# kvas7andy/unreal

Hardware: AMD Instinct MI355X
Metric: env-steps/sec (whole node), UNREAL maze 84x84 (higher is better)
Workload: dtype f32 (fp16x2-split MFMA operands, fp32 accumulate)

## Files before the change

include/unreal_hip.h:

```cpp
#ifndef UNREAL_HIP_H
#define UNREAL_HIP_H
#include <stdint.h>
#ifdef __cplusplus
extern "C" {
#endif

#define UNREAL_FRAME_BYTES 21168
#define UNREAL_PC_CELLS 400
#define UNREAL_GEMM_RELU 1
#define UNREAL_GEMM_ACCUM 2
#define UNREAL_GEMM_ATOMIC 4
#define UNREAL_GEMM_RELU_MASK 8
#define UNREAL_GEMM_RELU_BITS 16

#define UNREAL_MAZE_NAV_RECORD 8
#define UNREAL_MAZE_GEN_RECORD(N) (8 + 18 + (N) * (N) + 65)
#define UNREAL_MAZE_TOP_DOWN 0
#define UNREAL_MAZE_FIRST_PERSON 1
#define UNREAL_MAZE_FIRST_PERSON_GENERATED 2
int unreal_maze_reset(int B, int H1, const int* mask, int* pos, int* last_action, float* last_reward, const int* count,
                      uint8_t* frames, int view, int N, const int* cfg, int actor_base, int* goal, int* layout,
                      int* ep_steps, int* episode, int* heading, void* stream);
int unreal_maze_step(int B, int H1, const int* actions, const int* active, int* pos, int* last_action, float* last_reward,
                     int* count, uint8_t* frames, float* r_reward, int* r_action, int* r_terminal, int* r_last_action,
// ... 99 lines not shown
int unreal_gemm_f32_split_nt(int M, int N, int K, const float* A, int lda, const float* a_absmax, const uint16_t* W2,
                             int ldw, long plane_stride, const float* w_absmax, float* C, int ldc, float* c_absmax,
                             const float* bias,
                             const void* mask ,
                             int ldm, int flags, int splitk, void* stream);
int unreal_gemm_f32_split_nt_slabs(int M, int N, int K, const float* A, int lda, const float* a_absmax, const uint16_t* W3,
                                   int ldw, long plane_stride, const float* w_absmax, float* C, int ldc, float* c_absmax,
                                   const float* bias, int flags, int splitk, float* partials, long partial_floats,
                                   void* stream);
int unreal_gemm_f32_split_tn(int M, int N, int K, const float* A, int lda, const float* a_absmax, const float* B, int ldb,
                             const float* b_absmax, float* C, int ldc, float* colsum, int splitk, void* stream);
int unreal_shadow_refresh_multi(const void* abs_descs, int n_abs, int abs_blocks, const void* split_descs, int n_split,
                                int split_blocks, void* stream);
int unreal_split_f16x2(int rows, int cols, const float* src, int ld_src, int transpose, int row_perm, uint16_t* dst,
                       int ld_dst, long plane_stride, const float* w_absmax, void* stream);
int unreal_lstm_step_fwd(int rows, const float* x, int ldx, int Kx, const float* x_absmax, const float* h_prev, int ld_hprev,
                         const uint16_t* W2, int ldw, long plane_stride, const float* w_absmax, float* gates,
                         const float* bias, const float* c_prev, float* c_out, float* h_out, int ld_h, void* stream);
int unreal_lstm_bptt_step(int rows, const float* d_gates, const float* a_absmax, const uint16_t* Wh2, int ldw,
                          long plane_stride, const float* w_absmax, const float* dh_above, float* dc_io,
                          const float* gates_act, const float* c_prev, const float* c_new, float* dpre,
                          float* dpre_absmax0, float* dpre_absmax1, void* stream);
int unreal_lstm_gates_fwd(int rows, const float* pre, const float* bias, const float* c_prev, float* gates_act,
                          float* c_out, float* h_out, int ld_h, void* stream);
int unreal_lstm_gates_bwd(int rows, const float* dh_above, const float* dh_rec, float* dc_io, const float* gates_act,
                          const float* c_prev, const float* c_new, float* dpre, float* dpre_absmax0 ,
                          float* dpre_absmax1 , void* stream);

int unreal_linear_small_fwd(int rows, int K, int NOUT, const float* X, int ldx, const float* W, const float* b,
                            float* out, int ldo, void* stream);
int unreal_linear_small_bwd(int rows, int K, int NOUT, const float* X, int ldx, const float* dO, int ldo,
                            const float* W, float* dX, int lddx, int accumulate_dx, float* dW, int dw_stride_k,
                            int dw_stride_n, float* db, void* stream);
int unreal_softmax_sample(int rows, int A, float* logits_pi, int ld, const double* u, int* action, void* stream);
int unreal_policy_step(int rows, int A, const float* X, int ldx, const float* Wp, const float* bp, const float* Wv,
                       const float* bv, const double* u, float* pi_out, float* v_out, int* action, void* stream);
int unreal_base_loss_grad(int rows, int A, const float* pi, int ld_pi, const float* v, const int* action,
                          const float* adv, const float* R, const int* active, float entropy_beta, float grad_scale,
                          float* dlogits, float* dv, float* losses , void* stream);
int unreal_vr_loss_grad(int rows, const float* v, const float* R, const int* mask, float grad_scale, float* dv,
                        float* loss, void* stream);
int unreal_rp_loss_grad(int rows, const float* logits, const int* cls, float grad_scale, float* prob, float* dlogits,
                        float* loss, void* stream);
int unreal_colsum(int rows, int cols, const float* X, int ld, float* out, void* stream);
int unreal_relu_mask(int rows, int cols, float* d, int ldd, const float* src, int lds, void* stream);

int unreal_pc_deconv_fwd(int N, int A, const float* hp, const float* hp_absmax, const float* Wv, const float* bv,
                         const float* Wa, const float* ba, float* qmax, const int* action, const float* target,
                         const int* mask, float lambda, float grad_scale, float* d_dec, float* ddec_absmax, float* loss,
                         void* stream);
int unreal_pc_deconv_bwd(int N, int A, const float* hp, const float* hp_absmax, const float* d_dec, const float* ddec_absmax,
                         const float* Wv, const float* Wa, float* d_hp, float* dhp_absmax ,
                         float* dWv, float* dbv, float* dWa, float* dba, void* stream);
int unreal_pc_deconv_train(int N, int A, const float* hp, const float* hp_absmax, const float* Wv, const float* bv,
                           const float* Wa, const float* ba, const int* action, const float* target, const int* mask,
                           float lambda, float grad_scale, float* loss, float* d_hp,
                           float* dhp_absmax , float* dWv, float* dbv, float* dWa,
                           float* dba, float* d_dec, void* stream);

int unreal_grad_norm(const float* grad, long n, float* scratch , float* norm_out, void* stream);
int unreal_rmsprop_step(float* var, float* ms, float* mom, const float* grad, long n, float lr, float decay,
                        float momentum, float eps, float clip_norm, const float* norm, void* stream);

int unreal_copy_words(long n, const void* src, void* dst, void* stream);
int unreal_axpy_f32(long n, float alpha, const float* x, float* y, void* stream);
int unreal_last_launch(char* buf, int len, void* stream);
// ... 6 lines not shown
```

unreal_amd/csrc/heads.hip:

```cpp
#include "common.h"
#include "policy_row.h"

namespace {

__device__ __forceinline__ float sigmoidf_(float x) { return 1.f / (1.f + expf(-x)); }

__global__ void lstm_gates_fwd_kernel(int rows, const float* __restrict__ pre, const float* __restrict__ bias,
                                      const float* __restrict__ c_prev, float* __restrict__ gates_act,
                                      float* __restrict__ c_out, float* __restrict__ h_out, int ld_h) {
  int g = blockIdx.x * blockDim.x + threadIdx.x;
  if (g >= rows * LSTM_N) return;
  int r = g / LSTM_N, u = g - r * LSTM_N;
  const float* p = pre + (size_t)r * 4 * LSTM_N;
  float i = sigmoidf_(p[u] + bias[u]);
  float j = tanhf(p[LSTM_N + u] + bias[LSTM_N + u]);
  float f = sigmoidf_(p[2 * LSTM_N + u] + bias[2 * LSTM_N + u] + 1.0f);
  float o = sigmoidf_(p[3 * LSTM_N + u] + bias[3 * LSTM_N + u]);
  float c = c_prev[g] * f + i * j;
  float h = tanhf(c) * o;
  if (gates_act) {
    float* ga = gates_act + (size_t)r * 4 * LSTM_N;
    ga[u] = i; ga[LSTM_N + u] = j; ga[2 * LSTM_N + u] = f; ga[3 * LSTM_N + u] = o;
  }
  c_out[g] = c;
  h_out[(size_t)r * ld_h + u] = h;
}

__global__ void lstm_gates_bwd_kernel(int rows, const float* __restrict__ dh_above, const float* __restrict__ dh_rec,
                                      float* __restrict__ dc_io, const float* __restrict__ gates_act,
                                      const float* __restrict__ c_prev, const float* __restrict__ c_new,
                                      float* __restrict__ dpre, float* absmax0, float* absmax1) {
  float m = 0.f;
// ... 6 lines not shown
  float dc = dc_io[g] + dh * o * (1.f - tc * tc);
  float* d = dpre + (size_t)r * 4 * LSTM_N;
  const float d0 = dc * j * i * (1.f - i), d1 = dc * i * (1.f - j * j), d2 = dc * c_prev[g] * f * (1.f - f),
              d3 = dh * tc * o * (1.f - o);
  d[u] = d0;
  d[LSTM_N + u] = d1;
  d[2 * LSTM_N + u] = d2;
  d[3 * LSTM_N + u] = d3;
  dc_io[g] = dc * f;
  m = fmaxf(fmaxf(m, fmaxf(fabsf(d0), fabsf(d1))), fmaxf(fabsf(d2), fabsf(d3)));
  }
  __shared__ float wmx[4];
  m = wave_max(m);
  if ((threadIdx.x & 63) == 0) wmx[threadIdx.x >> 6] = m;
  __syncthreads();
  if (threadIdx.x < 64) {
    const float mm = fmaxf(fmaxf(wmx[0], wmx[1]), fmaxf(wmx[2], wmx[3]));
    absmax_commit(absmax0, mm);
    absmax_commit(absmax1, mm);
  }
}

template <int NOUT>
__global__ __launch_bounds__(256) void linear_small_fwd_kernel(int rows, int K, const float* __restrict__ X, int ldx,
                                                               const float* __restrict__ W, const float* __restrict__ b,
                                                               float* __restrict__ out, int ldo) {
  int row = blockIdx.x * 4 + (threadIdx.x >> 6);
  int lane = threadIdx.x & 63;
  if (row >= rows) return;
  float acc[NOUT];
#pragma unroll
  for (int n = 0; n < NOUT; ++n) acc[n] = 0.f;
  const float* x = X + (size_t)row * ldx;
  for (int k = lane; k < K; k += 64) {
    float xv = x[k];
#pragma unroll
    for (int n = 0; n < NOUT; ++n) acc[n] += xv * W[(size_t)k * NOUT + n];
  }
#pragma unroll
  for (int n = 0; n < NOUT; ++n) acc[n] = wave_sum(acc[n]);
  if (lane == 0)
#pragma unroll
    for (int n = 0; n < NOUT; ++n) out[(size_t)row * ldo + n] = acc[n] + b[n];
}

template <int NOUT>
__global__ __launch_bounds__(256) void linear_small_bwd_kernel(int rows, int K, int rows_per_block,
                                                               const float* __restrict__ X, int ldx,
                                                               const float* __restrict__ dO, int ldo,
                                                               const float* __restrict__ W, float* __restrict__ dX,
                                                               int lddx, int accumulate_dx, float* __restrict__ dW,
                                                               int dw_sk, int dw_sn, float* __restrict__ db) {
  const int k = blockIdx.x * 256 + threadIdx.x;
  const int r0 = blockIdx.y * rows_per_block;
  const int nr = min(rows_per_block, rows - r0);
  if (k >= K) return;
  float w[NOUT], acc[NOUT], sdb[NOUT];
#pragma unroll
  for (int n = 0; n < NOUT; ++n) { w[n] = W ? W[(size_t)k * NOUT + n] : 0.f; acc[n] = 0.f; sdb[n] = 0.f; }
  int r = 0;
  for (; r + 4 <= nr; r += 4) {
    float xv[4], old[4], d[4][NOUT];
#pragma unroll
    for (int u = 0; u < 4; ++u) xv[u] = X[(size_t)(r0 + r + u) * ldx + k];
    if (dX && accumulate_dx) {
#pragma unroll
      for (int u = 0; u < 4; ++u) old[u] = dX[(size_t)(r0 + r + u) * lddx + k];
    }
#pragma unroll
    for (int u = 0; u < 4; ++u)
// ... 2 lines not shown
#pragma unroll
    for (int u = 0; u < 4; ++u) {
      float dx = 0.f;
#pragma unroll
      for (int n = 0; n < NOUT; ++n) {
        acc[n] += xv[u] * d[u][n];
        dx += d[u][n] * w[n];
        sdb[n] += d[u][n];
      }
      if (dX) dX[(size_t)(r0 + r + u) * lddx + k] = accumulate_dx ? (old[u] + dx) : dx;
    }
  }
  for (; r < nr; ++r) {
    const size_t row = (size_t)(r0 + r);
    float xv = X[row * ldx + k];
    float dx = 0.f;
#pragma unroll
    for (int n = 0; n < NOUT; ++n) {
      const float d = dO[row * ldo + n];
      acc[n] += xv * d;
      dx += d * w[n];
      sdb[n] += d;
    }
    if (dX) {
      float* p = dX + row * lddx + k;
      *p = accumulate_dx ? (*p + dx) : dx;
    }
  }
#pragma unroll
  for (int n = 0; n < NOUT; ++n) atomicAdd(dW + (size_t)k * dw_sk + (size_t)n * dw_sn, acc[n]);
  if (db && k == 0) {
#pragma unroll
    for (int n = 0; n < NOUT; ++n) atomicAdd(db + n, sdb[n]);
  }
}

__global__ void softmax_sample_kernel(int rows, int A, float* __restrict__ logits_pi, int ld, const double* __restrict__ u,
                                      int* __restrict__ action) {
  int r = blockIdx.x * blockDim.x + threadIdx.x;
  if (r >= rows) return;
  float* p = logits_pi + (size_t)r * ld;
  float m = p[0];
  for (int a = 1; a < A; ++a) m = fmaxf(m, p[a]);
  float s = 0.f;
  for (int a = 0; a < A; ++a) { float e = expf(p[a] - m); p[a] = e; s += e; }
  for (int a = 0; a < A; ++a) p[a] = p[a] / s;
  if (action && u) {
    double tot = 0.0;
    for (int a = 0; a < A; ++a) tot += (double)p[a];
    double run = 0.0, uu = u[r];
    int act = 0;
    for (int a = 0; a < A; ++a) {
      run += (double)p[a];
      if (run / tot <= uu) act = a + 1;
    }
    action[r] = min(act, A - 1);
  } else if (action) {
    int best = 0;
    for (int a = 1; a < A; ++a)
      if (p[a] > p[best]) best = a;
    action[r] = best;
  }
}

template <int A>
__global__ __launch_bounds__(256) void policy_step_kernel(int rows, const float* __restrict__ X, int ldx,
// ... 114 lines not shown
  }
  part[ry][cx] = (s0 + s1) + (s2 + s3);
  __syncthreads();
  if (ry == 0 && c < cols) atomicAdd(out + c, (part[0][cx] + part[1][cx]) + (part[2][cx] + part[3][cx]));
}

__global__ void relu_mask_kernel(int rows, int cols, float* __restrict__ d, int ldd, const float* __restrict__ src, int lds) {
  int g = blockIdx.x * blockDim.x + threadIdx.x;
  if (g >= rows * cols) return;
  int r = g / cols, c = g - r * cols;
  float* p = d + (size_t)r * ldd + c;
  if (!(src[(size_t)r * lds + c] > 0.f)) *p = 0.f;
}

template <int NOUT>
int launch_small_fwd(int rows, int K, const float* X, int ldx, const float* W, const float* b, float* out, int ldo,
                     hipStream_t st) {
  hipLaunchKernelGGL((linear_small_fwd_kernel<NOUT>), dim3((rows + 3) / 4), dim3(256), 0, st, rows, K, X, ldx, W, b, out,
                     ldo);
  return unreal_launch_status();
}

template <int NOUT>
int launch_small_bwd(int rows, int K, const float* X, int ldx, const float* dO, int ldo, const float* W, float* dX,
                     int lddx, int acc, float* dW, int dw_sk, int dw_sn, float* db, hipStream_t st) {
  if (dw_sk == 0 && dw_sn == 0) { dw_sk = NOUT; dw_sn = 1; }
  const int rpb = 128;
  dim3 grid((K + 255) / 256, (rows + rpb - 1) / rpb);
  hipLaunchKernelGGL((linear_small_bwd_kernel<NOUT>), grid, dim3(256), 0, st, rows, K, rpb, X,
                     ldx, dO, ldo, W, dX, lddx, acc, dW, dw_sk, dw_sn, db);
  return unreal_launch_status();
}

}

#define GRID1(n) dim3(((n) + 255) / 256), dim3(256), 0, (hipStream_t)stream

extern "C" {

int unreal_lstm_gates_fwd(int rows, const float* pre, const float* bias, const float* c_prev, float* gates_act,
                          float* c_out, float* h_out, int ld_h, void* stream) {
  if (rows <= 0 || !pre || !bias || !c_prev || !c_out || !h_out || ld_h < LSTM_N) return UNREAL_EINVAL;
  hipLaunchKernelGGL(lstm_gates_fwd_kernel, GRID1(rows * LSTM_N), rows, pre, bias, c_prev, gates_act, c_out, h_out,
                     ld_h);
  return unreal_launch_status();
}

int unreal_lstm_gates_bwd(int rows, const float* dh_above, const float* dh_rec, float* dc_io, const float* gates_act,
                          const float* c_prev, const float* c_new, float* dpre, float* dpre_absmax0, float* dpre_absmax1,
                          void* stream) {
  if (rows <= 0 || !dh_above || !dc_io || !gates_act || !c_prev || !c_new || !dpre) return UNREAL_EINVAL;
  hipLaunchKernelGGL(lstm_gates_bwd_kernel, dim3(min(rows, 1024)), dim3(256), 0, (hipStream_t)stream, rows, dh_above, dh_rec,
                     dc_io, gates_act, c_prev, c_new, dpre, dpre_absmax0, dpre_absmax1);
  return unreal_launch_status();
}

int unreal_linear_small_fwd(int rows, int K, int NOUT, const float* X, int ldx, const float* W, const float* b,
                            float* out, int ldo, void* stream) {
  if (rows <= 0 || K <= 0 || !X || !W || !b || !out || ldx < K || ldo < NOUT) return UNREAL_EINVAL;
  hipStream_t st = (hipStream_t)stream;
  switch (NOUT) {
#define SMALL_FWD(n) case n: return launch_small_fwd<n>(rows, K, X, ldx, W, b, out, ldo, st);
    SMALL_FWD(1) SMALL_FWD(3) SMALL_FWD(4) SMALL_FWD(6)
    SMALL_FWD(2) SMALL_FWD(5) SMALL_FWD(7) SMALL_FWD(8) SMALL_FWD(9)
    SMALL_FWD(10) SMALL_FWD(11) SMALL_FWD(12) SMALL_FWD(13) SMALL_FWD(14) SMALL_FWD(15) SMALL_FWD(16) SMALL_FWD(17)
    SMALL_FWD(18) SMALL_FWD(19)
#undef SMALL_FWD
    default: return UNREAL_EINVAL;
  }
}

int unreal_linear_small_bwd(int rows, int K, int NOUT, const float* X, int ldx, const float* dO, int ldo,
                            const float* W, float* dX, int lddx, int accumulate_dx, float* dW, int dw_stride_k,
                            int dw_stride_n, float* db, void* stream) {
  if (rows <= 0 || K <= 0 || !X || !dO || !dW || ldx < K || ldo < NOUT) return UNREAL_EINVAL;
  if (dX && !W) return UNREAL_EINVAL;
  hipStream_t st = (hipStream_t)stream;
  switch (NOUT) {
#define SMALL_BWD(n) \
    case n: return launch_small_bwd<n>(rows, K, X, ldx, dO, ldo, W, dX, lddx, accumulate_dx, dW, dw_stride_k, dw_stride_n, db, st);
    SMALL_BWD(1) SMALL_BWD(3) SMALL_BWD(4) SMALL_BWD(5) SMALL_BWD(6) SMALL_BWD(7)
    SMALL_BWD(2) SMALL_BWD(8) SMALL_BWD(9) SMALL_BWD(10) SMALL_BWD(11) SMALL_BWD(12) SMALL_BWD(13)
    SMALL_BWD(14) SMALL_BWD(15) SMALL_BWD(16) SMALL_BWD(17) SMALL_BWD(18) SMALL_BWD(19)
#undef SMALL_BWD
    default: return UNREAL_EINVAL;
  }
}

int unreal_softmax_sample(int rows, int A, float* logits_pi, int ld, const double* u, int* action, void* stream) {
  if (rows <= 0 || A <= 0 || A > UNREAL_MAX_ACTIONS || !logits_pi || ld < A) return UNREAL_EINVAL;
  hipLaunchKernelGGL(softmax_sample_kernel, GRID1(rows), rows, A, logits_pi, ld, u, action);
  return unreal_launch_status();
}

int unreal_policy_step(int rows, int A, const float* X, int ldx, const float* Wp, const float* bp, const float* Wv,
                       const float* bv, const double* u, float* pi_out, float* v_out, int* action, void* stream) {
  if (rows <= 0 || !X || !Wp || !bp || !Wv || !bv || !pi_out || !v_out || !action || ldx < LSTM_N) return UNREAL_EINVAL;
  hipStream_t st = (hipStream_t)stream;
  dim3 grid((rows + 3) / 4), block(256);
  switch (A) {
#define POLICY_STEP(a) \
    case a: hipLaunchKernelGGL((policy_step_kernel<a>), grid, block, 0, st, rows, X, ldx, Wp, bp, Wv, bv, u, pi_out, v_out, action); break;
    POLICY_STEP(3) POLICY_STEP(4) POLICY_STEP(6)
    POLICY_STEP(2) POLICY_STEP(5) POLICY_STEP(7) POLICY_STEP(8) POLICY_STEP(9) POLICY_STEP(10)
    POLICY_STEP(11) POLICY_STEP(12) POLICY_STEP(13) POLICY_STEP(14) POLICY_STEP(15) POLICY_STEP(16) POLICY_STEP(17)
    POLICY_STEP(18)
#undef POLICY_STEP
    default: return UNREAL_EINVAL;
  }
  return unreal_launch_status();
}

int unreal_base_loss_grad(int rows, int A, const float* pi, int ld_pi, const float* v, const int* action,
                          const float* adv, const float* R, const int* active, float entropy_beta, float grad_scale,
                          float* dlogits, float* dv, float* losses, void* stream) {
  if (rows <= 0 || A <= 0 || A > UNREAL_MAX_ACTIONS || !pi || !v || !action || !adv || !R || !active || !dlogits || !dv ||
      !losses)
    return UNREAL_EINVAL;
  if (A <= 8)
    hipLaunchKernelGGL(base_loss_grad_kernel<8>, GRID1(rows), rows, A, pi, ld_pi, v, action, adv, R, active, entropy_beta,
                       grad_scale, dlogits, dv, losses);
// ... 36 lines not shown
```

unreal_amd/csrc/replay.hip:

```cpp
#include "common.h"

namespace {

__global__ void sample_seq_kernel(int B, int H, int H1, int L, const int* start_draw, const int* count,
                                  const int* r_terminal, int* seq_idx, int* seq_len) {
  int b = blockIdx.x * blockDim.x + threadIdx.x;
  if (b >= B) return;
  const int cnt = count[b];
  const int top = max(0, cnt - H);
  int a0 = top + start_draw[b];
  const size_t rb = (size_t)b * H1;
  if (r_terminal[rb + a0 % H1]) a0 += 1;
  int n = 0, last = 0;
  for (int i = 0; i < L; ++i) {
    int a = min(a0 + i, cnt - 1);
    int idx = (int)(rb + a % H1);
    seq_idx[(size_t)i * B + b] = idx;
    last = idx;
    ++n;
    if (r_terminal[idx]) break;
  }
  for (int i = n; i < L; ++i) seq_idx[(size_t)i * B + b] = last;
  seq_len[b] = n;
}
// ... 33 lines not shown
    int pc = __popcll(m);
    if (run + pc > rank) {
      int k = rank - run;
      int before = __popcll(m & ((1ull << lane) - 1ull));
      unsigned long long hit = __ballot(member && before == k);
      end = lo + c + (__ffsll((long long)hit) - 1);
      break;
    }
    run += pc;
  }
  if (lane < 3) rp_idx[b * 3 + lane] = (int)(rb + (end - 3 + lane) % H1);
  if (lane == 0) {
    float r = r_reward[rb + end % H1];
    rp_class[b] = (r > -1e-10f && r < 1e-10f) ? 0 : (r > 0.f ? 1 : 2);
  }
}

__global__ void base_returns_kernel(int B, int T, const float* rewards, const float* values, const int* n_steps,
                                    const float* boot_v, const int* terminal_end, double gamma, float* R_out,
                                    float* adv_out) {
  int b = blockIdx.x * blockDim.x + threadIdx.x;
  if (b >= B) return;
  const int n = n_steps[b];
  double R = terminal_end[b] ? 0.0 : (double)boot_v[b];
  for (int t = T - 1; t >= 0; --t) {
    size_t i = (size_t)t * B + b;
    if (t >= n) { R_out[i] = 0.f; adv_out[i] = 0.f; continue; }
    R = (double)rewards[i] + gamma * R;
    R_out[i] = (float)R;
    adv_out[i] = (float)(R - (double)values[i]);
  }
}

__global__ void vr_returns_kernel(int B, int L, const int* seq_idx, const int* seq_len, const float* r_reward,
                                  const int* r_terminal, const float* boot_v, double gamma, float* R_out) {
  int b = blockIdx.x * blockDim.x + threadIdx.x;
  if (b >= B) return;
  const int n = seq_len[b];
  double R = (n >= 2 && r_terminal[seq_idx[(size_t)(n - 2) * B + b]]) ? 0.0 : (double)boot_v[b];
  for (int t = L - 2; t >= 0; --t) {
    size_t i = (size_t)t * B + b;
    if (t >= n - 1) { R_out[i] = 0.f; continue; }
    R = (double)r_reward[seq_idx[i]] + gamma * R;
    R_out[i] = (float)R;
  }
}

__global__ void pc_returns_kernel(int B, int L, const int* seq_idx, const int* seq_len, const float* r_pc,
                                  const int* r_terminal, const float* boot_qmax, double gamma_pc, float* R_out) {
  int g = blockIdx.x * blockDim.x + threadIdx.x;
  if (g >= B * PC_CELLS) return;
  const int b = g / PC_CELLS, c = g - b * PC_CELLS;
  const int n = seq_len[b];
  double R = (n >= 2 && r_terminal[seq_idx[(size_t)(n - 2) * B + b]]) ? 0.0 : (double)boot_qmax[g];
  for (int t = L - 2; t >= 0; --t) {
    size_t row = (size_t)t * B + b;
    if (t >= n - 1) { R_out[row * PC_CELLS + c] = 0.f; continue; }
    R = (double)r_pc[(size_t)seq_idx[row] * PC_CELLS + c] + gamma_pc * R;
    R_out[row * PC_CELLS + c] = (float)R;
  }
}

__global__ void lar_fill_kernel(int rows, int A, const int* last_action, const float* last_reward, const int* idx,
                                float* xcat, int ld, int col0, int clip) {
  int g = blockIdx.x * blockDim.x + threadIdx.x;
  const int w = ld - col0;
  if (g >= rows * w) return;
  int r = g / w, k = g - r * w;
  int src = idx ? idx[r] : r;
  float v = 0.f;
  if (k < A) v = (last_action[src] == k) ? 1.f : 0.f;
  else if (k == A) v = clip ? fminf(fmaxf(last_reward[src], -1.f), 1.f) : last_reward[src];
  xcat[(size_t)r * ld + col0 + k] = v;
}

__global__ void objective_put_kernel(int B, int H1, int obj, const int* count, const int* active, const float* staged,
                                     float* r_objective) {
  int g = blockIdx.x * blockDim.x + threadIdx.x;
  if (g >= B * obj) return;
  int b = g / obj, j = g - b * obj;
  if (active && !active[b]) return;
  r_objective[((size_t)b * H1 + count[b] % H1) * obj + j] = staged[g];
}

__global__ void objective_fill_kernel(int rows, int obj, int H1, const float* r_objective, const int* idx, int slot_offset,
                                      float* xcat, int ld, int col0) {
  int g = blockIdx.x * blockDim.x + threadIdx.x;
  if (g >= rows * obj) return;
  int r = g / obj, j = g - r * obj;
  int f = idx[r], b = f / H1, s = f - b * H1;
  s = (s + slot_offset % H1 + H1) % H1;
  xcat[(size_t)r * ld + col0 + j] = r_objective[((size_t)b * H1 + s) * obj + j];
// ... 178 lines not shown
```

unreal_amd/ops.py:

```python
import torch

from ._lib import lib, ptr, stream

FRAME_BYTES = 21168
PC_CELLS = 400
F2_DIM = 2592
C1_DIM = 6400
GEMM_RELU, GEMM_ACCUM, GEMM_ATOMIC, GEMM_RELU_MASK, GEMM_RELU_BITS = 1, 2, 4, 8, 16
RELU_WORDS = 162

FRAME_SHAPE = (84, 84)
FRAME_HW_MIN, FRAME_HW_MAX = 20, 480


def frame_dims(H, W):
    H, W = int(H), int(W)
    if not (FRAME_HW_MIN <= H <= FRAME_HW_MAX and FRAME_HW_MIN <= W <= FRAME_HW_MAX):
        raise ValueError("frame size %dx%d: supported are %d <= H, W <= %d" % (H, W, FRAME_HW_MIN, FRAME_HW_MAX))
    h1, w1 = (H - 8) // 4 + 1, (W - 8) // 4 + 1
    h2, w2 = (h1 - 4) // 2 + 1, (w1 - 4) // 2 + 1
    return h1, w1, h2, w2, 32 * h2 * w2


def frame_stride(H, W):
# ... 712 lines not shown


def lstm_bptt_step(rows, d_gates, Wh, dh_above, dc_io, gates_act, c_prev, c_new, dpre, a_max=None, c_max0=None,
                   c_max1=None):
    if Wh.N != 256 or Wh.K != 1024 or getattr(Wh, "row_perm", 0):
        raise ValueError("lstm_bptt_step needs the natural [256,1024] shadow of the recurrent kernel rows")
    _chk(d_gates, "f32", rows * 1024, "d_gates"); _chk(dh_above, "f32", rows * 256); _chk(dc_io, "f32", rows * 256)
    _chk(gates_act, "f32", rows * 1024); _chk(c_prev, "f32", rows * 256); _chk(c_new, "f32", rows * 256)
    _chk(dpre, "f32", rows * 1024)
    _chk(a_max, "f32", 1, "a_max", optional=True); _chk(c_max0, "f32", 1, "c_max0", optional=True)
    _chk(c_max1, "f32", 1, "c_max1", optional=True)
    a_max = _absmax_of(d_gates, rows, 1024, 1024, a_max)
    _call("unreal_lstm_bptt_step", rows, ptr(d_gates), ptr(a_max), ptr(Wh.planes), Wh.ldw, Wh.plane, ptr(Wh.wmax),
          ptr(dh_above), ptr(dc_io), ptr(gates_act), ptr(c_prev), ptr(c_new), ptr(dpre), ptr(c_max0), ptr(c_max1))


def linear_small_fwd(rows, K, NOUT, X, ldx, W, b, out, ldo):
    _chk(X, "f32", (rows - 1) * ldx + K); _chk(W, "f32", K * NOUT); _chk(b, "f32", NOUT)
    _chk(out, "f32", (rows - 1) * ldo + NOUT)
    _call("unreal_linear_small_fwd", rows, K, NOUT, ptr(X), ldx, ptr(W), ptr(b), ptr(out), ldo)


def linear_small_bwd(rows, K, NOUT, X, ldx, dO, ldo, W, dX, lddx, accumulate_dx, dW, db, dw_stride_k=0, dw_stride_n=0):
    _chk(X, "f32", (rows - 1) * ldx + K); _chk(dO, "f32", (rows - 1) * ldo + NOUT)
    _chk(W, "f32", K * NOUT, optional=dX is None)
    _chk(dX, "f32", (rows - 1) * lddx + K, optional=True)
    sk, sn = (dw_stride_k, dw_stride_n) if (dw_stride_k or dw_stride_n) else (NOUT, 1)
    _chk(dW, "f32", (K - 1) * sk + (NOUT - 1) * sn + 1)
    _chk(db, "f32", NOUT, optional=True)
    _call("unreal_linear_small_bwd", rows, K, NOUT, ptr(X), ldx, ptr(dO), ldo, ptr(W), ptr(dX), lddx,
          int(accumulate_dx), ptr(dW), int(dw_stride_k), int(dw_stride_n), ptr(db))


def policy_step(rows, A, X, ldx, Wp, bp, Wv, bv, u, pi_out, v_out, action):
    _chk(X, "f32", (rows - 1) * ldx + 256, "X"); _chk(Wp, "f32", 256 * A); _chk(bp, "f32", A); _chk(Wv, "f32", 256)
    _chk(bv, "f32", 1); _chk(u, "f64", rows, "u", optional=True); _chk(pi_out, "f32", rows * A); _chk(v_out, "f32", rows)
    _chk(action, "i32", rows)
    _call("unreal_policy_step", rows, A, ptr(X), ldx, ptr(Wp), ptr(bp), ptr(Wv), ptr(bv), ptr(u), ptr(pi_out), ptr(v_out),
          ptr(action))


def softmax_sample(rows, A, logits_pi, ld, u=None, action=None):
    _chk(logits_pi, "f32", (rows - 1) * ld + A); _chk(u, "f64", rows, optional=True)
    _chk(action, "i32", rows, optional=True)
    _call("unreal_softmax_sample", rows, A, ptr(logits_pi), ld, ptr(u), ptr(action))


def base_loss_grad(rows, A, pi, ld_pi, v, action, adv, R, active, beta, grad_scale, dlogits, dv, losses):
    _chk(pi, "f32", (rows - 1) * ld_pi + A); _chk(v, "f32", rows); _chk(action, "i32", rows)
    _chk(adv, "f32", rows); _chk(R, "f32", rows); _chk(active, "i32", rows)
    _chk(dlogits, "f32", rows * A); _chk(dv, "f32", rows); _chk(losses, "f32", 3)
    _call("unreal_base_loss_grad", rows, A, ptr(pi), ld_pi, ptr(v), ptr(action), ptr(adv), ptr(R), ptr(active),
          float(beta), float(grad_scale), ptr(dlogits), ptr(dv), ptr(losses))


def vr_loss_grad(rows, v, R, mask, grad_scale, dv, loss):
    _chk(v, "f32", rows); _chk(R, "f32", rows); _chk(mask, "i32", rows); _chk(dv, "f32", rows); _chk(loss, "f32", 1)
    _call("unreal_vr_loss_grad", rows, ptr(v), ptr(R), ptr(mask), float(grad_scale), ptr(dv), ptr(loss))


def rp_loss_grad(rows, logits, cls, grad_scale, prob, dlogits, loss):
    _chk(logits, "f32", rows * 3); _chk(cls, "i32", rows); _chk(prob, "f32", rows * 3, optional=True)
    _chk(dlogits, "f32", rows * 3); _chk(loss, "f32", 1)
    _call("unreal_rp_loss_grad", rows, ptr(logits), ptr(cls), float(grad_scale), ptr(prob), ptr(dlogits), ptr(loss))


# ... 75 lines not shown
```

unreal_amd/train/trainer.py:

```python
import time

import torch

from .. import ops
from ..environment.environment import Environment
from ..environment.maze_environment import batched_maze_environment
from ..model.model import UnrealModel, PathWS, GradWS
from .experience import Experience

PERFORMANCE_LOG_INTERVAL = 2000


def log_uniform(lo, hi, rate):
    import math
    return math.exp(math.log(lo) * (1 - rate) + math.log(hi) * rate)


class PhiloxDraws(object):

    def __init__(self, seed, rank=0, batch=None, world_size=1):
        self.seed = int(seed)
        self.counter = 1
        self.batch = None if batch is None else int(batch)
        self.stride = None if batch is None else int(batch) * int(world_size)
# ... 384 lines not shown
                    nxt = dict(next_idx=ws.frame_idx[(t + 1) * B:(t + 2) * B])
                    if self.use_lstm:
                        nxt.update(next_lar=ws.xcat[(t + 1) * B * ws.xld:], lar_ld=ws.xld, lar_col0=256, A=A)
                if fuse_policy:
                    self.environment.policy_rollout_step(net, feat, ld, self.u_act[s], self.pi[t * B * A:(t + 1) * B * A],
                                                         self.v[s], self.actions[s], self.rewards[s], self.terminals[s],
                                                         self.active, self.active_log[s], self.n_steps, self.terminal_end,
                                                         **nxt)
                    continue
                self.environment.rollout_step(self.actions[s], self.rewards[s], self.terminals[s], self.active,
                                              self.active_log[s], self.n_steps, self.terminal_end, **nxt)
                continue
            self.environment.process(self.actions[s], self.active, self.rewards[s], self.terminals[s],
                                     reset_on_terminal=True, track_score=True)
            ops.rollout_advance(B, self.terminals[s], self.active, self.active_log[s], self.n_steps,
                                self.terminal_end)
        if self.use_lstm:
            ops.copy_(self.lstm_c, ws.c[(T - 1) * B * 256:T * B * 256])
            ops.copy_(self.lstm_h, ws.h[(T - 1) * B * 256:T * B * 256])
        bw = self.boot_ws
        if self.use_lstm:
            ops.copy_(bw.c0, self.lstm_c)
            ops.copy_(bw.h0, self.lstm_h)
        self.ring.cur_idx(out=bw.frame_idx[:B])
        feat, ld = net.trunk_forward(self.ring, bw, 1, B, lar_from_ring=False, save_c1=False,
                                     clip_lar=self.rp_mode == 1,
                                     objective_slot_offset=-1)
        net.value_forward(B, feat, ld, self.boot_v)
        if self.use_lstm:
            ops.reset_state(B, self.terminal_end, self.lstm_c, self.lstm_h)
        ops.base_returns(B, T, self.rewards, self.v, self.n_steps, self.boot_v, self.terminal_end, self.gamma,
                         self.R, self.adv)

    def _train_base(self):
        B, T, A, ws, net, g, p = self.Bg, self.n_step_TD, self.action_size, self.base_ws, self.local_network, \
            self.local_network.g, self.local_network.p
        rows = T * B
        ops.base_loss_grad(rows, A, self.pi, A, self.v, self.actions, self.adv, self.R, self.active_log,
                           self.entropy_beta, self.grad_scale, self.dlogits, self.dv, self.losses[0:3])
        feat, ld = net.features(ws)
        d_feat = self.gws.d_feat
        ops.linear_small_bwd(rows, 256, A, feat, ld, self.dlogits, A, p["W_base_fc_p"], d_feat, 256, False,
                             g["W_base_fc_p"], g["b_base_fc_p"])
        ops.linear_small_bwd(rows, 256, 1, feat, ld, self.dv, 1, p["W_base_fc_v"], d_feat, 256, True,
                             g["W_base_fc_v"], g["b_base_fc_v"])
        net.trunk_backward(self.ring, ws, self.gws, T, B, d_feat, h0_nonzero=True)

    def _sample_sequence(self):
        B, Ta, net = self.Bg, self.local_t_max, self.local_network
        L = Ta + 1
        self.draws.randint(self.experience_history_size - L - 1, self.seq_start)
        ops.replay_sample_seq(self.ring, L, self.seq_start, self.seq_idx, self.seq_len)
        bw = self.boot_ws
        ops.seq_last_idx(B, self.seq_idx, self.seq_len, bw.frame_idx[:B])
        if self.use_lstm:
            bw.c0.zero_()
            bw.h0.zero_()
        feat, ld = net.trunk_forward(self.ring, bw, 1, B, lar_from_ring=True, save_c1=False)
        return feat, ld

    def _aux_forward(self):
        B, Ta, net, ws = self.Bg, self.local_t_max, self.local_network, self.aux_ws
        rows = Ta * B
        ops.copy_(ws.frame_idx[:rows], self.seq_idx[:rows])
        if self.use_lstm:
            ws.c0.zero_()
            ws.h0.zero_()
        ops.seq_mask(B, Ta, self.seq_len, self.seq_mask)
        return net.trunk_forward(self.ring, ws, Ta, B, lar_from_ring=True, save_c1=True)

    fuse_pc_deconv = True
    keep_d_dec = False

    def _pc_deconv_loss_backward(self, gws, rows, mask, d_hp, s_hp):
        A, net = self.action_size, self.local_network
        p, g = net.p, net.g
        s_dhp = net.new_slot()
        if self.fuse_pc_deconv:
# ... 64 lines not shown
            ops.replay_sample_seq(self.ring, L, self.seq_start2[s], self.seq_idx2[s], self.seq_len2[s])
            ops.seq_last_idx(B, self.seq_idx2[s], self.seq_len2[s], self.last2[s * B:(s + 1) * B])
            ops.seq_mask(B, Ta, self.seq_len2[s], self.seq_mask2[s])
        bw = self.boot2_ws
        ops.gather_i32(self.last2, self.map_boot, bw.frame_idx[:2 * B])
        feat, ld = net.trunk_forward(self.ring, bw, 1, 2 * B, lar_from_ring=True, save_c1=False)
        s_bhp = net.new_slot()
        net.pc_head_forward(B, feat, 2 * ld, self.boot_hp, ws=self.boot2_ws, hp_max=s_bhp)
        ops.pc_deconv_fwd(B, A, self.boot_hp, p["W_pc_deconv_v"], p["b_pc_deconv_v"], p["W_pc_deconv_a"],
                          p["b_pc_deconv_a"], qmax=self.boot_qmax, hp_max=s_bhp)
        ops.pc_returns(self.ring, L, self.seq_idx2[0], self.seq_len2[0], self.boot_qmax, self.gamma_pc, gws.pc_R)
        net.value_forward(B, feat[ld:], 2 * ld, self.aux_boot_v)
        ops.vr_returns(self.ring, L, self.seq_idx2[1], self.seq_len2[1], self.aux_boot_v, self.gamma, self.aux_R)
        ws = self.aux2_ws
        ops.gather_i32(self.seq_idx_cat, self.map_seq, ws.frame_idx[:2 * rows])
        feat, ld = net.trunk_forward(self.ring, ws, Ta, 2 * B, lar_from_ring=True, save_c1=True)
        d_feat = gws.d_feat
        s_hp = net.new_slot()
        net.pc_head_forward(rows, feat, 2 * ld, gws.hp, ws=self.aux2_ws, hp_max=s_hp)
        ops.gather_i32(self.ring.r_action, self.seq_idx2[0][:rows], self.seq_act)
        d_hp = gws.d_hp
        s_dhp = self._pc_deconv_loss_backward(gws, rows, self.seq_mask2[0], d_hp, s_hp)
        from ..model.model import _splitk
        ops.gemm_split_tn(256, 2592, rows, feat, 2 * ld, d_hp, 2592, g["W_pc_fc1"], 2592,
                          splitk=_splitk(256, 2592, rows), colsum=g["b_pc_fc1"],
                          a_max=net._one if self.use_lstm else self.aux2_ws.s_x, b_max=s_dhp)
        ops.gemm_split_nt(rows, 256, 2592, d_hp, 2592, sh["pc_fc1_dgrad"], d_feat, 2 * 256, a_max=s_dhp)
        net.value_forward(rows, feat[ld:], 2 * ld, self.aux_v)
        ops.vr_loss_grad(rows, self.aux_v, self.aux_R, self.seq_mask2[1], self.grad_scale, self.aux_dv, self.losses[4:5])
        ops.linear_small_bwd(rows, 256, 1, feat[ld:], 2 * ld, self.aux_dv, 1, p["W_base_fc_v"], d_feat[256:], 2 * 256, False,
                             g["W_base_fc_v"], g["b_base_fc_v"])
        net.trunk_backward(self.ring, ws, gws, Ta, 2 * B, d_feat)

    def _train_rp(self):
        B, net, ws = self.Bg, self.local_network, self.rp_ws
        p, g, gws = net.p, net.g, self.gws
        self.draws.randint(2, self.rp_coin)
        self.draws.uniform(self.rp_u)
        ops.replay_sample_rp(self.ring, self.rp_coin, self.rp_u, ws.frame_idx[:3 * B], self.rp_class, self.rp_mode)
        s_c1 = net.new_slot()
        F = net.F
        net.encoder_forward(self.ring, ws.frame_idx[:3 * B], ws.f2, ws.c1, c1_max=s_c1, ws=ws)
        ops.linear_small_fwd(B, 3 * F, 3, ws.f2, 3 * F, p["W_rp_fc1"], p["b_rp_fc1"], self.rp_logits, 3)
        ops.rp_loss_grad(B, self.rp_logits, self.rp_class, self.grad_scale, None, self.rp_dlogits,
                         self.losses[5:6])
        ops.linear_small_bwd(B, 3 * F, 3, ws.f2, 3 * F, self.rp_dlogits, 3, p["W_rp_fc1"], gws.d_f2, 3 * F, False,
                             g["W_rp_fc1"], g["b_rp_fc1"])
        ops.relu_mask(3 * B, F, gws.d_f2, F, ws.f2, F)
        net.encoder_backward(self.ring, ws.frame_idx[:3 * B], ws.c1, gws.d_f2,
                             c1_max=s_c1)

    def compute_gradients(self):
        net = self.local_network
        net.refresh_shadows()
        net.begin_pass()
        self._rollout()
        net.grads.flat.zero_()
        self.losses.zero_()
        self._train_base()
        if self.batch_aux:
            self._train_aux_batched()
        else:
            if self.use_pixel_change:
                self._train_pc()
            if self.use_value_replay:
                self._train_vr()
        if self.use_reward_prediction:
            self._train_rp()

    def process(self, sess=None, global_t=0, summary_writer=None, summary_op_dict=None, score_input=None,
                sr_input=None, eval_input=None, entropy_input=None, term_global_t=None, losses_input=None,
                sync_stats=True):
        if self.environment is None:
            self.prepare()
        if not self._full:
            self._fill_experience(sess)
            return 0, None
        net = self.local_network
# ... 63 lines not shown
```

Before: 3.711 million.

## Fuse small-head backward passes, unroll linear_small_fwd, and prefetch returns loads

Adds a one-pass small-linear backward kernel. It computes the policy and value head gradients together, and for the reward-prediction head it folds in the ReLU mask and the dx absmax. Both trainer paths are switched to it by default. This removes separate launches and repeated reads of the features. The forward small-linear loop is also unrolled with grouped loads. The returns kernels now prefetch chunks of reward loads before running the serial recurrence. The risks are changed fp summation order in dx and a new dependency on encoder_backward accepting a d2_max argument.

```diff
diff --git a/include/unreal_hip.h b/include/unreal_hip.h
--- a/include/unreal_hip.h
+++ b/include/unreal_hip.h
@@ -155,6 +155,12 @@
 int unreal_linear_small_bwd(int rows, int K, int NOUT, const float* X, int ldx, const float* dO, int ldo,
                             const float* W, float* dX, int lddx, int accumulate_dx, float* dW, int dw_stride_k,
                             int dw_stride_n, float* db, void* stream);
+int unreal_linear_small_bwd2(int rows, int K, int n1, int n2, const float* X, int ldx, const float* dO1, int ldo1,
+                             const float* W1, float* dW1, float* db1 , const float* dO2, int ldo2,
+                             const float* W2, float* dW2, float* db2 , float* dX, int lddx, void* stream);
+int unreal_linear_small_bwd_relu(int rows, int K, int NOUT, const float* X, int ldx, const float* dO, int ldo,
+                                 const float* W, float* dX, int lddx, float* dW, float* db ,
+                                 float* dx_absmax, void* stream);
 int unreal_softmax_sample(int rows, int A, float* logits_pi, int ld, const double* u, int* action, void* stream);
 int unreal_policy_step(int rows, int A, const float* X, int ldx, const float* Wp, const float* bp, const float* Wv,
                        const float* bv, const double* u, float* pi_out, float* v_out, int* action, void* stream);
diff --git a/unreal_amd/csrc/heads.hip b/unreal_amd/csrc/heads.hip
--- a/unreal_amd/csrc/heads.hip
+++ b/unreal_amd/csrc/heads.hip
@@ -1,3 +1,5 @@
+#include <type_traits>
+
 #include "common.h"
 #include "policy_row.h"
 
@@ -70,10 +72,25 @@
 #pragma unroll
   for (int n = 0; n < NOUT; ++n) acc[n] = 0.f;
   const float* x = X + (size_t)row * ldx;
-  for (int k = lane; k < K; k += 64) {
+  constexpr int U = NOUT <= 4 ? 8 : (NOUT <= 8 ? 4 : 1);
+  int k = lane;
+  for (; k + (U - 1) * 64 < K; k += U * 64) {
+    float xv[U], wv[U][NOUT];
+#pragma unroll
+    for (int u = 0; u < U; ++u) xv[u] = x[k + 64 * u];
+#pragma unroll
+    for (int u = 0; u < U; ++u)
+#pragma unroll
+      for (int n = 0; n < NOUT; ++n) wv[u][n] = W[(size_t)(k + 64 * u) * NOUT + n];
+#pragma unroll
+    for (int u = 0; u < U; ++u)
+#pragma unroll
+      for (int n = 0; n < NOUT; ++n) acc[n] = __builtin_fmaf(xv[u], wv[u][n], acc[n]);
+  }
+  for (; k < K; k += 64) {
     float xv = x[k];
 #pragma unroll
-    for (int n = 0; n < NOUT; ++n) acc[n] += xv * W[(size_t)k * NOUT + n];
+    for (int n = 0; n < NOUT; ++n) acc[n] = __builtin_fmaf(xv, W[(size_t)k * NOUT + n], acc[n]);
   }
 #pragma unroll
   for (int n = 0; n < NOUT; ++n) acc[n] = wave_sum(acc[n]);
@@ -142,6 +159,111 @@
   if (db && k == 0) {
 #pragma unroll
     for (int n = 0; n < NOUT; ++n) atomicAdd(db + n, sdb[n]);
+  }
+}
+
+template <int N, bool TAIL_ROW>
+__device__ __forceinline__ float small_bwd_dx(const float* d, const float* w) {
+#pragma clang fp contract(off)
+  constexpr int NF = TAIL_ROW ? N : (N > 12 ? N - 12 : 0);
+  float dx = 0.f;
+#pragma unroll
+  for (int n = 0; n < N; ++n) {
+    if (n < NF) {
+      dx = __builtin_fmaf(d[n], w[n], dx);
+    } else {
+      const float p = d[n] * w[n];
+      dx = dx + p;
+    }
+  }
+  return dx;
+}
+
+template <int N1, int N2, bool RELU>
+__global__ __launch_bounds__(256) void linear_small_bwd_1pass_kernel(
+    int rows, int K, int rows_per_block, const float* __restrict__ X, int ldx, const float* __restrict__ dO1, int ldo1,
+    const float* __restrict__ W1, float* __restrict__ dW1, float* __restrict__ db1, const float* __restrict__ dO2, int ldo2,
+    const float* __restrict__ W2, float* __restrict__ dW2, float* __restrict__ db2, float* __restrict__ dX, int lddx,
+    float* dx_absmax) {
+  constexpr int M2 = N2 ? N2 : 1;
+  const int k = blockIdx.x * 256 + threadIdx.x;
+  const bool live = k < K;
+  const int kc = live ? k : K - 1;
+  const int r0 = blockIdx.y * rows_per_block;
+  const int nr = min(rows_per_block, rows - r0);
+  float w1[N1], acc1[N1], sdb1[N1], w2[M2], acc2[M2], sdb2[M2];
+#pragma unroll
+  for (int n = 0; n < N1; ++n) { w1[n] = W1[(size_t)kc * N1 + n]; acc1[n] = 0.f; sdb1[n] = 0.f; }
+#pragma unroll
+  for (int n = 0; n < M2; ++n) { w2[n] = N2 ? W2[(size_t)kc * N2 + n] : 0.f; acc2[n] = 0.f; sdb2[n] = 0.f; }
+  float m = 0.f;
+  auto trip = [&](int r, auto U_, auto TAIL_) {
+    constexpr int U = decltype(U_)::value;
+    constexpr bool TAIL_ROW = decltype(TAIL_)::value;
+    float xv[U], d1[U][N1], d2[U][M2];
+#pragma unroll
+    for (int u = 0; u < U; ++u) xv[u] = X[(size_t)(r0 + r + u) * ldx + kc];
+#pragma unroll
+    for (int u = 0; u < U; ++u) {
+#pragma unroll
+      for (int n = 0; n < N1; ++n) d1[u][n] = dO1[(size_t)(r0 + r + u) * ldo1 + n];
+#pragma unroll
+      for (int n = 0; n < M2; ++n) d2[u][n] = N2 ? dO2[(size_t)(r0 + r + u) * ldo2 + n] : 0.f;
+    }
+#pragma unroll
+    for (int u = 0; u < U; ++u) {
+#pragma unroll
+      for (int n = 0; n < N1; ++n) {
+        acc1[n] += xv[u] * d1[u][n];
+        sdb1[n] += d1[u][n];
+      }
+      float dx = small_bwd_dx<N1, TAIL_ROW>(d1[u], w1);
+      if (N2) {
+#pragma unroll
+        for (int n = 0; n < M2; ++n) {
+          acc2[n] += xv[u] * d2[u][n];
+          sdb2[n] += d2[u][n];
+        }
+        dx = dx + small_bwd_dx<M2, TAIL_ROW>(d2[u], w2);
+      }
+      if (RELU) {
+        dx = xv[u] > 0.f ? dx : 0.f;
+        m = fmaxf(m, fabsf(dx));
+      }
+      if (live) dX[(size_t)(r0 + r + u) * lddx + k] = dx;
+    }
+  };
+  const std::false_type body;
+  const std::true_type tail;
+  const int n_body = min(nr, (rows & ~3) - r0);
+  int r = 0;
+  for (; r + 8 <= n_body; r += 8) trip(r, std::integral_constant<int, 8>(), body);
+  for (; r < n_body; ++r) trip(r, std::integral_constant<int, 1>(), body);
+  for (; r < nr; ++r) trip(r, std::integral_constant<int, 1>(), tail);
+  if (live) {
+#pragma unroll
+    for (int n = 0; n < N1; ++n) atomicAdd(dW1 + (size_t)k * N1 + n, acc1[n]);
+    if (N2) {
+#pragma unroll
+      for (int n = 0; n < M2; ++n) atomicAdd(dW2 + (size_t)k * N2 + n, acc2[n]);
+    }
+  }
+  if (k == 0) {
+    if (db1) {
+#pragma unroll
+      for (int n = 0; n < N1; ++n) atomicAdd(db1 + n, sdb1[n]);
+    }
+    if (N2 && db2) {
+#pragma unroll
+      for (int n = 0; n < M2; ++n) atomicAdd(db2 + n, sdb2[n]);
+    }
+  }
+  if (RELU) {
+    __shared__ float wmx[4];
+    m = wave_max(live ? m : 0.f);
+    if ((threadIdx.x & 63) == 0) wmx[threadIdx.x >> 6] = m;
+    __syncthreads();
+    if (threadIdx.x < 64) absmax_commit(dx_absmax, fmaxf(fmaxf(wmx[0], wmx[1]), fmaxf(wmx[2], wmx[3])));
   }
 }
 
@@ -322,6 +444,17 @@
   return unreal_launch_status();
 }
 
+template <int N1, int N2, bool RELU>
+int launch_small_bwd_1pass(int rows, int K, const float* X, int ldx, const float* dO1, int ldo1, const float* W1, float* dW1,
+                           float* db1, const float* dO2, int ldo2, const float* W2, float* dW2, float* db2, float* dX,
+                           int lddx, float* dx_absmax, hipStream_t st) {
+  const int rpb = 64;
+  dim3 grid((K + 255) / 256, (rows + rpb - 1) / rpb);
+  hipLaunchKernelGGL((linear_small_bwd_1pass_kernel<N1, N2, RELU>), grid, dim3(256), 0, st, rows, K, rpb, X, ldx, dO1, ldo1,
+                     W1, dW1, db1, dO2, ldo2, W2, dW2, db2, dX, lddx, dx_absmax);
+  return unreal_launch_status();
+}
+
 }
 
 #define GRID1(n) dim3(((n) + 255) / 256), dim3(256), 0, (hipStream_t)stream
@@ -377,6 +510,34 @@
   }
 }
 
+int unreal_linear_small_bwd2(int rows, int K, int n1, int n2, const float* X, int ldx, const float* dO1, int ldo1,
+                             const float* W1, float* dW1, float* db1, const float* dO2, int ldo2, const float* W2,
+                             float* dW2, float* db2, float* dX, int lddx, void* stream) {
+  if (rows <= 0 || K <= 0 || !X || !dO1 || !W1 || !dW1 || !dO2 || !W2 || !dW2 || !dX || ldx < K || lddx < K ||
+      ldo1 < n1 || ldo2 < n2)
+    return UNREAL_EINVAL;
+  if (n2 != 1) return UNREAL_EINVAL;
+  hipStream_t st = (hipStream_t)stream;
+  switch (n1) {
+#define SMALL_BWD2(n) \
+    case n: return launch_small_bwd_1pass<n, 1, false>(rows, K, X, ldx, dO1, ldo1, W1, dW1, db1, dO2, ldo2, W2, dW2, db2, dX, lddx, nullptr, st);
+    SMALL_BWD2(1) SMALL_BWD2(2) SMALL_BWD2(3) SMALL_BWD2(4) SMALL_BWD2(5) SMALL_BWD2(6) SMALL_BWD2(7) SMALL_BWD2(8) SMALL_BWD2(9)
+    SMALL_BWD2(10) SMALL_BWD2(11) SMALL_BWD2(12) SMALL_BWD2(13) SMALL_BWD2(14) SMALL_BWD2(15) SMALL_BWD2(16) SMALL_BWD2(17)
+    SMALL_BWD2(18)
+#undef SMALL_BWD2
+    default: return UNREAL_EINVAL;
+  }
+}
+
+int unreal_linear_small_bwd_relu(int rows, int K, int NOUT, const float* X, int ldx, const float* dO, int ldo,
+                                 const float* W, float* dX, int lddx, float* dW, float* db, float* dx_absmax, void* stream) {
+  if (rows <= 0 || K <= 0 || !X || !dO || !W || !dX || !dW || !dx_absmax || ldx < K || lddx < K || ldo < NOUT)
+    return UNREAL_EINVAL;
+  if (NOUT != 3) return UNREAL_EINVAL;
+  return launch_small_bwd_1pass<3, 0, true>(rows, K, X, ldx, dO, ldo, W, dW, db, nullptr, 0, nullptr, nullptr, nullptr, dX,
+                                            lddx, dx_absmax, (hipStream_t)stream);
+}
+
 int unreal_softmax_sample(int rows, int A, float* logits_pi, int ld, const double* u, int* action, void* stream) {
   if (rows <= 0 || A <= 0 || A > UNREAL_MAX_ACTIONS || !logits_pi || ld < A) return UNREAL_EINVAL;
   hipLaunchKernelGGL(softmax_sample_kernel, GRID1(rows), rows, A, logits_pi, ld, u, action);
diff --git a/unreal_amd/csrc/replay.hip b/unreal_amd/csrc/replay.hip
--- a/unreal_amd/csrc/replay.hip
+++ b/unreal_amd/csrc/replay.hip
@@ -89,32 +89,58 @@
   }
 }
 
-__global__ void vr_returns_kernel(int B, int L, const int* seq_idx, const int* seq_len, const float* r_reward,
-                                  const int* r_terminal, const float* boot_v, double gamma, float* R_out) {
+#define RET_CH 20
+
+__global__ void vr_returns_kernel(int B, int L, const int* __restrict__ seq_idx, const int* __restrict__ seq_len,
+                                  const float* __restrict__ r_reward, const int* __restrict__ r_terminal,
+                                  const float* __restrict__ boot_v, double gamma, float* __restrict__ R_out) {
   int b = blockIdx.x * blockDim.x + threadIdx.x;
   if (b >= B) return;
   const int n = seq_len[b];
   double R = (n >= 2 && r_terminal[seq_idx[(size_t)(n - 2) * B + b]]) ? 0.0 : (double)boot_v[b];
-  for (int t = L - 2; t >= 0; --t) {
-    size_t i = (size_t)t * B + b;
-    if (t >= n - 1) { R_out[i] = 0.f; continue; }
-    R = (double)r_reward[seq_idx[i]] + gamma * R;
-    R_out[i] = (float)R;
-  }
-}
-
-__global__ void pc_returns_kernel(int B, int L, const int* seq_idx, const int* seq_len, const float* r_pc,
-                                  const int* r_terminal, const float* boot_qmax, double gamma_pc, float* R_out) {
+  for (int t1 = L - 2; t1 >= 0; t1 -= RET_CH) {
+    float v[RET_CH];
+#pragma unroll
+    for (int u = 0; u < RET_CH; ++u) {
+      const int t = t1 - u;
+      v[u] = r_reward[seq_idx[(size_t)min(max(t, 0), max(n - 2, 0)) * B + b]];
+    }
+#pragma unroll
+    for (int u = 0; u < RET_CH; ++u) {
+      const int t = t1 - u;
+      if (t < 0) break;
+      size_t i = (size_t)t * B + b;
+      if (t >= n - 1) { R_out[i] = 0.f; continue; }
+      R = (double)v[u] + gamma * R;
+      R_out[i] = (float)R;
+    }
+  }
+}
+
+__global__ void pc_returns_kernel(int B, int L, const int* __restrict__ seq_idx, const int* __restrict__ seq_len,
+                                  const float* __restrict__ r_pc, const int* __restrict__ r_terminal,
+                                  const float* __restrict__ boot_qmax, double gamma_pc, float* __restrict__ R_out) {
   int g = blockIdx.x * blockDim.x + threadIdx.x;
   if (g >= B * PC_CELLS) return;
   const int b = g / PC_CELLS, c = g - b * PC_CELLS;
   const int n = seq_len[b];
   double R = (n >= 2 && r_terminal[seq_idx[(size_t)(n - 2) * B + b]]) ? 0.0 : (double)boot_qmax[g];
-  for (int t = L - 2; t >= 0; --t) {
-    size_t row = (size_t)t * B + b;
-    if (t >= n - 1) { R_out[row * PC_CELLS + c] = 0.f; continue; }
-    R = (double)r_pc[(size_t)seq_idx[row] * PC_CELLS + c] + gamma_pc * R;
-    R_out[row * PC_CELLS + c] = (float)R;
+  for (int t1 = L - 2; t1 >= 0; t1 -= RET_CH) {
+    float v[RET_CH];
+#pragma unroll
+    for (int u = 0; u < RET_CH; ++u) {
+      const int t = t1 - u;
+      v[u] = r_pc[(size_t)seq_idx[(size_t)min(max(t, 0), max(n - 2, 0)) * B + b] * PC_CELLS + c];
+    }
+#pragma unroll
+    for (int u = 0; u < RET_CH; ++u) {
+      const int t = t1 - u;
+      if (t < 0) break;
+      size_t row = (size_t)t * B + b;
+      if (t >= n - 1) { R_out[row * PC_CELLS + c] = 0.f; continue; }
+      R = (double)v[u] + gamma_pc * R;
+      R_out[row * PC_CELLS + c] = (float)R;
+    }
   }
 }
 
diff --git a/unreal_amd/ops.py b/unreal_amd/ops.py
--- a/unreal_amd/ops.py
+++ b/unreal_amd/ops.py
@@ -768,6 +768,24 @@
           int(accumulate_dx), ptr(dW), int(dw_stride_k), int(dw_stride_n), ptr(db))
 
 
+def linear_small_bwd2(rows, K, n1, n2, X, ldx, dO1, ldo1, W1, dW1, db1, dO2, ldo2, W2, dW2, db2, dX, lddx):
+    _chk(X, "f32", (rows - 1) * ldx + K); _chk(dX, "f32", (rows - 1) * lddx + K)
+    for n, dO, ldo, W, dW, db in ((n1, dO1, ldo1, W1, dW1, db1), (n2, dO2, ldo2, W2, dW2, db2)):
+        _chk(dO, "f32", (rows - 1) * ldo + n); _chk(W, "f32", K * n); _chk(dW, "f32", K * n)
+        _chk(db, "f32", n, optional=True)
+    _call("unreal_linear_small_bwd2", rows, K, n1, n2, ptr(X), ldx, ptr(dO1), ldo1, ptr(W1), ptr(dW1), ptr(db1),
+          ptr(dO2), ldo2, ptr(W2), ptr(dW2), ptr(db2), ptr(dX), lddx)
+
+
+def linear_small_bwd_relu(rows, K, NOUT, X, ldx, dO, ldo, W, dX, lddx, dW, db, dx_max):
+    _chk(X, "f32", (rows - 1) * ldx + K); _chk(dO, "f32", (rows - 1) * ldo + NOUT); _chk(W, "f32", K * NOUT)
+    _chk(dX, "f32", (rows - 1) * lddx + K); _chk(dW, "f32", K * NOUT); _chk(db, "f32", NOUT, optional=True)
+    _chk(dx_max, "f32", 1, "dx_max")
+    _call("unreal_linear_small_bwd_relu", rows, K, NOUT, ptr(X), ldx, ptr(dO), ldo, ptr(W), ptr(dX), lddx, ptr(dW),
+          ptr(db), ptr(dx_max))
+    return dx_max
+
+
 def policy_step(rows, A, X, ldx, Wp, bp, Wv, bv, u, pi_out, v_out, action):
     _chk(X, "f32", (rows - 1) * ldx + 256, "X"); _chk(Wp, "f32", 256 * A); _chk(bp, "f32", A); _chk(Wv, "f32", 256)
     _chk(bv, "f32", 1); _chk(u, "f64", rows, "u", optional=True); _chk(pi_out, "f32", rows * A); _chk(v_out, "f32", rows)
diff --git a/unreal_amd/train/trainer.py b/unreal_amd/train/trainer.py
--- a/unreal_amd/train/trainer.py
+++ b/unreal_amd/train/trainer.py
@@ -440,6 +440,8 @@
         ops.base_returns(B, T, self.rewards, self.v, self.n_steps, self.boot_v, self.terminal_end, self.gamma,
                          self.R, self.adv)
 
+    fuse_base_heads = True
+
     def _train_base(self):
         B, T, A, ws, net, g, p = self.Bg, self.n_step_TD, self.action_size, self.base_ws, self.local_network, \
             self.local_network.g, self.local_network.p
@@ -448,10 +450,15 @@
                            self.entropy_beta, self.grad_scale, self.dlogits, self.dv, self.losses[0:3])
         feat, ld = net.features(ws)
         d_feat = self.gws.d_feat
-        ops.linear_small_bwd(rows, 256, A, feat, ld, self.dlogits, A, p["W_base_fc_p"], d_feat, 256, False,
-                             g["W_base_fc_p"], g["b_base_fc_p"])
-        ops.linear_small_bwd(rows, 256, 1, feat, ld, self.dv, 1, p["W_base_fc_v"], d_feat, 256, True,
-                             g["W_base_fc_v"], g["b_base_fc_v"])
+        if self.fuse_base_heads:
+            ops.linear_small_bwd2(rows, 256, A, 1, feat, ld, self.dlogits, A, p["W_base_fc_p"], g["W_base_fc_p"],
+                                  g["b_base_fc_p"], self.dv, 1, p["W_base_fc_v"], g["W_base_fc_v"], g["b_base_fc_v"],
+                                  d_feat, 256)
+        else:
+            ops.linear_small_bwd(rows, 256, A, feat, ld, self.dlogits, A, p["W_base_fc_p"], d_feat, 256, False,
+                                 g["W_base_fc_p"], g["b_base_fc_p"])
+            ops.linear_small_bwd(rows, 256, 1, feat, ld, self.dv, 1, p["W_base_fc_v"], d_feat, 256, True,
+                                 g["W_base_fc_v"], g["b_base_fc_v"])
         net.trunk_backward(self.ring, ws, self.gws, T, B, d_feat, h0_nonzero=True)
 
     def _sample_sequence(self):
@@ -582,6 +589,8 @@
                              g["W_base_fc_v"], g["b_base_fc_v"])
         net.trunk_backward(self.ring, ws, gws, Ta, 2 * B, d_feat)
 
+    fuse_rp_mask = True
+
     def _train_rp(self):
         B, net, ws = self.Bg, self.local_network, self.rp_ws
         p, g, gws = net.p, net.g, self.gws
@@ -594,6 +603,11 @@
         ops.linear_small_fwd(B, 3 * F, 3, ws.f2, 3 * F, p["W_rp_fc1"], p["b_rp_fc1"], self.rp_logits, 3)
         ops.rp_loss_grad(B, self.rp_logits, self.rp_class, self.grad_scale, None, self.rp_dlogits,
                          self.losses[5:6])
+        if self.fuse_rp_mask:
+            s_df2 = ops.linear_small_bwd_relu(B, 3 * F, 3, ws.f2, 3 * F, self.rp_dlogits, 3, p["W_rp_fc1"], gws.d_f2, 3 * F,
+                                              g["W_rp_fc1"], g["b_rp_fc1"], net.new_slot())
+            net.encoder_backward(self.ring, ws.frame_idx[:3 * B], ws.c1, gws.d_f2, c1_max=s_c1, d2_max=s_df2)
+            return
         ops.linear_small_bwd(B, 3 * F, 3, ws.f2, 3 * F, self.rp_dlogits, 3, p["W_rp_fc1"], gws.d_f2, 3 * F, False,
                              g["W_rp_fc1"], g["b_rp_fc1"])
         ops.relu_mask(3 * B, F, gws.d_f2, F, ws.f2, F)
```

Measured after the change: 3.566 million. -3.9%, worse.
